# mpitid/babble

Hardware: AMD Instinct MI355X
Metric: consensus-ordered events/sec at N participants (higher is better)
Workload: dtype int32; 1 GPU; random-gossip DAG, 256 participants, 10000000 events per GPU, RunConsensus every K=256 events (39063 calls); participants=256, events_per_graph=10000000, k=256, graphs_per_gpu=1, parallelism=replicas1

## Files before the change

### babble_amd/csrc/hge_coords.hip

```cpp
#include <hip/hip_runtime.h>
#include <stdint.h>

namespace hge {

__global__ void k_la_clear(Tables t, const int32_t* olen, const int32_t* len, int32_t* zero,
                           int nzero) {
  const int j = blockIdx.y;
  const int N = t.N;
  if (j == 0 && blockIdx.x == 0)
    for (int i = threadIdx.x; i < nzero; i += blockDim.x) zero[i] = 0;
  const int64_t lo = (int64_t)olen[j] * N, hi = (int64_t)len[j] * N;
  int32_t* base = t.LA + (size_t)j * t.ccap * N;
  for (int64_t e = lo + (int64_t)blockIdx.x * blockDim.x + threadIdx.x; e < hi;
       e += (int64_t)gridDim.x * blockDim.x)
    base[e] = -1;
}

template <int NP>
__global__ void __launch_bounds__(256) k_la_sweep(Tables t, const int2* segs, int nseg, int SEG,
                                                  const int32_t* len, const int32_t* prev,
                                                  int32_t* changed) {
  constexpr int G = 256 / NP;
  constexpr int SEGMAX = 64;
  constexpr int U = 32;
// ... 443 lines not shown
    for (int h = 0; h < 16; h += CH) {
      int kv[CH];
#pragma unroll
      for (int i = 0; i < CH; i++) {
        const int jj = c0 + ty + 4 * (h + i), q = p0 + tx;
        if (jj < N && q < pend) {
          const FT f = FDT[((size_t)jj * N + a) * ccap + q];
          kv[i] = (sizeof(FT) == 2 && f == (FT)0xFFFF) ? INF32 : (int)f;
        } else {
          kv[i] = INF32;
        }
      }
      int64_t tv[CH];
      const bool tson = p0 + tx >= ts0 && p0 + tx < ts1;
#pragma unroll
      for (int i = 0; i < CH; i++) {
        const int jj = c0 + ty + 4 * (h + i);
        tv[i] = tson ? t.tsch[(size_t)(jj < N ? jj : 0) * ccap + (kv[i] != INF32 ? kv[i] : 0)] : own;
      }
#pragma unroll
      for (int i = 0; i < CH; i++) {
        tile[ty + 4 * (h + i)][tx] = kv[i];
        const int64_t d = tv[i] - own;
        const bool esc = d < -(int64_t)INT32_MAX || d > (int64_t)INT32_MAX;
        toff[ty + 4 * (h + i)][tx] = kv[i] == INF32 ? 0 : (esc ? INT32_MIN : (int32_t)d);
      }
    }
    }
    __syncthreads();
    const int NT = (N + 63) >> 6;
    for (int r = ty; r < 64; r += 4) {
      const int q = p0 + r, jj = c0 + tx;
      const bool tsrow = q >= ts0 && q < ts1;
      bool esc = false;
      if (q < pend && jj < N) {
        const size_t o = rowoff(t, a, q) + jj;
        const int32_t dv = toff[tx][r];
        esc = dv == INT32_MIN;
        if constexpr (sizeof(FT) == 2) {
          const int f = tile[tx][r];
          __builtin_nontemporal_store((uint16_t)(f == INF32 ? 0xFFFFu : (uint32_t)f + 1), t.FD16 + o);
        } else {
          __builtin_nontemporal_store(tile[tx][r], t.FD + o);
        }
        if (tsrow) __builtin_nontemporal_store(dv, t.FDTD + o);
      }
      const bool any = __ballot(esc) != 0;
      if (tx == 0 && q < pend && tsrow) t.FDTW[((size_t)a * ccap + q) * NT + by] = any ? 1 : 0;
    }
    __syncthreads();
  }
}

__global__ void k_fdt16_to32(const uint16_t* src, int32_t* dst, size_t n, int bias) {
  for (size_t i = (size_t)blockIdx.x * blockDim.x + threadIdx.x; i < n; i += (size_t)gridDim.x * blockDim.x)
    dst[i] = src[i] == 0xFFFFu ? INF32 : (int32_t)src[i] - bias;
}

__global__ void __launch_bounds__(256) k_fd_qlo(Tables t, const int32_t* olen, const int32_t* len, int32_t* qlo) {
  fd_qlo_body(t, olen, len, qlo, blockIdx.x);
}
__global__ void __launch_bounds__(256) k_chain_fill_qlo(Tables t, int n0, int n1, const UpEv* up, UpDst dst, int nfb,
                                                        const int32_t* olen, const int32_t* len, int32_t* qlo,
                                                        int32_t* fst, int32_t* zbar, uint64_t* zgran, int ngran) {
  if (fst && blockIdx.x == gridDim.x - 1) {
    frontier_start_body(t, olen, len, fst, nullptr, zbar, zgran, ngran);
  } else if ((int)blockIdx.x < nfb) {
    const int x = n0 + blockIdx.x * blockDim.x + threadIdx.x;
    if (x < n1) chain_fill_one(t, x, n0, up, dst);
  } else {
    fd_qlo_body(t, olen, len, qlo, blockIdx.x - nfb);
  }
}

}
```

### babble_amd/csrc/hge_engine.hip

```cpp
#include <hip/hip_runtime.h>

#include <algorithm>
#include <chrono>
#include <cstdio>
#include <cstdlib>
#include <cstring>
#include <mutex>
#include <optional>
#include <string>
#include <thread>
#include <utility>
#include <vector>

#include "../../include/hge.h"
#include "hge_plan.h"
#include "hge_kernels.hip"
#include "hge_wide32.hip"
#include "hge_coords.hip"
#include "hge_coords_win.hip"
#include "hge_rounds_coop.hip"
#include "hge_rounds_direct.hip"
#include "hge_walk_spec.hip"

using namespace hge;

#define HIPCHK(x)                                                                    \
  do {                                                                               \
    hipError_t e_ = (x);                                                             \
    if (e_ != hipSuccess) {                                                          \
      throw EngineError(HGE_ERR_DEVICE, std::string(#x) + ": " + hipGetErrorString(e_)); \
    }                                                                                \
  } while (0)

#define KLAUNCH_AS(name, kern, ...)                                                    \
  do {                                                                                 \
    hp.launches++;                                                                     \
    prof_begin(name);                                                                  \
    hipLaunchKernelGGL(kern, __VA_ARGS__);                                             \
    const hipError_t le_ = hipGetLastError();                                          \
    if (le_ != hipSuccess)                                                             \
      throw EngineError(HGE_ERR_DEVICE, std::string("launch ") + name + ": " + hipGetErrorString(le_)); \
    prof_end();                                                                        \
  } while (0)
#define KLAUNCH(kern, ...) KLAUNCH_AS(#kern, kern, __VA_ARGS__)

#define NW_T(B, kern, ...) KLAUNCH(kern<B>, __VA_ARGS__)
#define NW_PT(B, kern, ...) KLAUNCH((kern<B>), __VA_ARGS__)
#define NW_PAT(B, kern, A, ...) KLAUNCH((kern<A, B>), __VA_ARGS__)
#define NW_PATC(B, kern, A, C, ...) KLAUNCH((kern<A, B, C>), __VA_ARGS__)
#define NW_SWITCH_(nw, CASE1, SHAPE, ...)                          \
  switch (nw) {                                                    \
    CASE1                                                          \
    case 2:                                                        \
      SHAPE(2, __VA_ARGS__);                                       \
      break;                                                       \
    case 3:                                                        \
      SHAPE(3, __VA_ARGS__);                                       \
      break;                                                       \
    case 4:                                                        \
      SHAPE(4, __VA_ARGS__);                                       \
      break;                                                       \
    default:                                                       \
      throw EngineError(HGE_ERR_INTERNAL, "unsupported N");        \
  }
#define KLAUNCH_NW(nw, SHAPE, ...) NW_SWITCH_(nw, case 1 : SHAPE(1, __VA_ARGS__); break;, SHAPE, __VA_ARGS__)
#define KLAUNCH_NW2(nw, SHAPE, ...) NW_SWITCH_(nw, , SHAPE, __VA_ARGS__)

namespace {

// ... 88 lines not shown
    pin_ord = nullptr;
    pin_ord_dev = nullptr;
    pin_ord_cap = 0;
    HIPCHK(hipHostMalloc((void**)&pin_ord, std::max<size_t>(n, 1) * 4, hipHostMallocDefault));
    pin_ord_cap = std::max<size_t>(n, 1);
    void* dp = nullptr;
    pin_ord_dev = hipHostGetDevicePointer(&dp, pin_ord, 0) == hipSuccess ? (int32_t*)dp : nullptr;
  }
  int64_t n_und = 0;

  std::vector<int64_t> replay_calls;
  std::vector<int64_t> replay_counts;

  int64_t Ecap = 0;
  int ccap = 0, Rcap = 0;
  DBuf<int32_t> d_creator, d_index, d_sp, d_op, d_ntx, d_round, d_rr, d_und;
  DBuf<int64_t> d_ts, d_cts;
  DBuf<uint64_t> d_S;
  DBuf<uint8_t> d_coin, d_wit;
  DBuf<int32_t> d_chain, d_LA, d_FD, d_FSS;
  DBuf<int32_t> s_w32, s_w32a;
  DBuf<uint32_t> d_LA16;
  DBuf<int2> d_opcp;
  DBuf<int64_t> d_tsch;
  DBuf<int32_t> d_C, d_W, d_rcnt, d_minw;
  DBuf<uint64_t> d_ssb, d_seeb;
  DBuf<uint8_t> d_fame;
  DBuf<int32_t> s_small, s_newwit;
  DBuf<int32_t> s_LCR, s_clast;
  DBuf<uint8_t> s_dec, s_decbit;
  DBuf<int32_t> s_segcnt, s_segcall, s_seground, s_theta;
  DBuf<uint8_t> s_segdec;
  DBuf<uint64_t> s_segfws;
  DBuf<int32_t> s_recv, s_rr, s_fund, s_upos, s_und2, s_bpos, s_vis;
  bool vis_all = false;
  DBuf<int64_t> s_cts;
  DBuf<unsigned char> s_keys, s_keys2;
  DBuf<int32_t> s_part, s_fst, s_relay, s_rfail;
  DBuf<uint8_t> s_dec2;
  bool minw_full = true;
  int n_sweeps = 0;
  DBuf<int32_t> d_FDT, s_chg, s_bar, s_dirty;
  DBuf<int32_t> s_src;
  DBuf<int4> s_lwplan;
  DBuf<uint32_t> s_lwsum, s_lwinit;
  DBuf<int32_t> s_lwpos, s_lwrisky;
  int ncu_cache = 0;
  int n_cu() {
    if (!ncu_cache) HIPCHK(hipDeviceGetAttribute(&ncu_cache, hipDeviceAttributeMultiprocessorCount, device));
    return ncu_cache;
  }
  DBuf<int32_t> d_FDTD;
  DBuf<uint8_t> d_FDTW;
  DBuf<int32_t> d_WLA;
  DBuf<uint16_t> d_WLR;
  DBuf<uint64_t> d_ssc, s_gran;
  DBuf<int32_t> s_bseg;
  DBuf<uint64_t> s_H;
  DBuf<int32_t> s_hn, s_hres;
  uint32_t walk_epoch = 0;
  int walk_chk[2] = {448, 2};
  bool coop_checked = false;
  int coop_nb = 0, coop_ncu = 0, coop_spec_nb = -1, coop_spec_bs = 0;
  const void* coop_spec_fn() const {
    return coop_spec_bs == 1024 ? (const void*)k_rounds_coop_spec<1024> : (const void*)k_rounds_coop_spec<512>;
  }
  DBuf<uint64_t> s_cH, s_cS, s_cT, s_cM;
  DBuf<uint32_t> s_mb;
  DBuf<int32_t> s_cn;
  uint32_t coop_epoch = 0;

  hipEvent_t ev[8] = {};
  bool prof_on = false;
  std::vector<hipEvent_t> prof_pool;
  std::vector<std::pair<std::string, int>> prof_rec;
  std::vector<std::string> prof_names;
  std::vector<double> prof_ms;
  std::vector<int64_t> prof_cnt;
  int R_div = 0;
  std::vector<int32_t> h_minw;
  DBuf<int32_t> s_cctl, s_out;
  std::vector<int32_t> h_cctl;
  int64_t* c_nc = nullptr;
  int32_t *c_Rc = nullptr, *c_Lc = nullptr, *c_flags = nullptr, *c_pr = nullptr, *c_pidx = nullptr;
  int32_t* c_sgo = nullptr;
  const int32_t* segoff_p = nullptr;
  DBuf<int32_t> s_kctl;
  std::vector<int32_t> h_kctl;
  std::vector<hge_plan::Seg> h_segs;
  bool und_fresh = false;
  float stage_ms[7] = {};

  Tables tables() const {
    Tables t;
    t.N = N;
    t.NW = NW;
    t.SM = SM;
    t.ccap = ccap;
    t.Rcap = Rcap;
    t.creator = d_creator.p;
    t.index = d_index.p;
    t.sp = d_sp.p;
    t.op = d_op.p;
    t.ts = d_ts.p;
    t.S = d_S.p;
    t.coin = d_coin.p;
// ... 69 lines not shown
      while (k < prof_names.size() && prof_names[k] != r.first) k++;
      if (k == prof_names.size()) {
        prof_names.push_back(r.first);
        prof_ms.push_back(0);
        prof_cnt.push_back(0);
      }
      prof_ms[k] += ms;
      prof_cnt[k] += 1;
    }
    prof_rec.clear();
  }

  DBuf<uint64_t> s_dbg;
  bool dbg_on = getenv("HGE_STAMPS") != nullptr;
  uint64_t* dbg_p() {
    if (!dbg_on) return nullptr;
    if (!s_dbg.p) {
      s_dbg.need(16);
      HIPCHK(hipMemset(s_dbg.p, 0, 16 * 8));
    }
    return s_dbg.p;
  }
  void dbg_dump() {
    if (!dbg_on || !s_dbg.p) return;
    uint64_t v[16];
    readback(v, s_dbg.p, 16);
    fprintf(stderr, "[hge stamps]");
    for (int i = 0; i < 16; i++) fprintf(stderr, " %llu", (unsigned long long)v[i]);
    fprintf(stderr, "\n");
  }

  void destroy() {
    if (st) (void)hipStreamSynchronize(st);
    if (getenv("HGE_HOST_PHASES") && hp.calls) {
      const double c = (double)hp.calls;
      fprintf(stderr,
              "{\"hge_host_phases\": {\"calls\": %lld, \"launches_per_call\": %.2f, \"copies_per_call\": %.2f, "
              "\"insert_us\": %.2f, \"consensus_us\": %.2f, \"sync_wait_us\": %.2f}}\n",
              (long long)hp.calls, hp.launches / c, hp.copies / c, hp.insert_ns / c / 1e3, hp.call_ns / c / 1e3,
              hp.wait_ns / c / 1e3);
    }
    for (auto& e : ev)
      if (e) (void)hipEventDestroy(e);
    for (auto& e : prof_pool) (void)hipEventDestroy(e);
    prof_pool.clear();
    DBuf<int32_t>* i32s[] = {&d_creator, &d_index,  &d_sp,    &d_op,     &d_ntx,     &d_round,
                             &d_rr,      &d_und,    &d_chain, &d_LA,     &d_FD,      &d_C,
                             &d_W,       &d_rcnt,   &d_minw,  &s_small,  &s_newwit,  &s_LCR,
                             &s_clast,   &s_segcnt, &s_segcall, &s_seground, &s_theta,
                             &s_recv,    &s_rr,     &s_bpos,  &s_fund,   &s_upos,    &s_vis,
                             &s_und2,    &s_part,   &s_fst,    &d_FSS,
                             &d_FDT,     &s_chg,    &s_bar,   &s_bseg,   &s_kctl,    &s_cctl,
                             &s_out,     &s_hn,     &s_hres,  &s_dirty,  &d_WLA,     &s_lwpos,
                             &s_lwrisky, &s_src,    &s_relay, &s_rfail};
    for (auto* b : i32s) b->free_();
    s_dec2.free_();
    s_lwplan.free_();
    d_WLR.free_();
    s_xbuf.free_();
    s_sord.free_();
    s_soff.free_();
    s_lwsum.free_();
    s_lwinit.free_();
    d_ts.free_();
    d_FDTD.free_();
    d_FDTW.free_();
    d_cts.free_();
    s_cts.free_();
    d_S.free_();
    d_ssb.free_();
    d_seeb.free_();
    s_H.free_();
    s_wdbg.free_();
    s_segfws.free_();
    d_coin.free_();
    d_wit.free_();
    d_fame.free_();
    s_dec.free_();
    s_decbit.free_();
    s_segdec.free_();
    s_keys.free_();
    s_keys2.free_();
    d_opcp.free_();
    d_tsch.free_();
    d_LA16.free_();
    d_ssc.free_();
    s_gran.free_();
    s_cH.free_();
    s_cS.free_();
    s_cT.free_();
    s_cM.free_();
    s_cn.free_();
    s_mb.free_();
    s_hist.free_();
    s_hstate.free_();
    s_hssc.free_();
    if (pin) (void)hipHostFree(pin);
    pin = nullptr;
    pin_cap = pin_used = 0;
    if (pin_ord) (void)hipHostFree(pin_ord);
    pin_ord = nullptr;
    pin_ord_dev = nullptr;
    pin_ord_cap = 0;
    cons_pin_n = 0;
    if (st) (void)hipStreamDestroy(st);
    st = nullptr;
  }
// ... 333 lines not shown
    if (!bytes) return;
    char* q = pin_take(bytes);
    hp.copies++;
    HIPCHK(hipMemcpyAsync(q, dev, bytes, hipMemcpyDeviceToHost, st));
    pending.push_back({host, (size_t)(q - pin), bytes});
  }
  size_t d2h_pinned(const void* dev, size_t bytes) {
    char* q = pin_take(bytes);
    if (bytes) hp.copies++;
    if (bytes) HIPCHK(hipMemcpyAsync(q, dev, bytes, hipMemcpyDeviceToHost, st));
    return (size_t)(q - pin);
  }
  int64_t n_syncs = 0;
  struct HostPhases {
    int64_t calls = 0, launches = 0, copies = 0, wait_ns = 0, call_ns = 0, insert_ns = 0;
  } hp;
  static int64_t now_ns() {
    return std::chrono::duration_cast<std::chrono::nanoseconds>(
               std::chrono::steady_clock::now().time_since_epoch()).count();
  }
  void sync() {
    n_syncs++;
    const int64_t w0 = now_ns();
    HIPCHK(hipStreamSynchronize(st));
    hp.wait_ns += now_ns() - w0;
    for (const Pending& pd : pending) memcpy(pd.dst, pin + pd.off, pd.bytes);
    pending.clear();
    pin_used = 0;
  }
  template <typename F>
  void readback(F* host, const F* dev, size_t n) {
    d2h(host, dev, n * sizeof(F));
    sync();
  }

  struct CoordStep {
    bool fresh = false;
    int64_t n0 = 0, n1 = 0;
    int maxnew = 0;
    int tot0 = 0;
    int SEG = 0, nseg = 0;
    int maxlen = 0, minlen = 0;
    enum class La { Windows, Seq, Sweeps } la = La::Sweeps;
    int32_t *rstate = nullptr, *olen = nullptr, *len = nullptr, *plo = nullptr, *qlo = nullptr;
    int32_t *fss_lo = nullptr, *fss_off = nullptr, *fss_total = nullptr, *segbase = nullptr;
    const int2* segs = nullptr;
    int32_t *cand_lo = nullptr, *cand_hi = nullptr;
    int32_t* risky1 = nullptr;
    const UpEv* up = nullptr;
    UpDst up_dst{};
    bool frontier_started = false;
    bool qlo_done = false;
    bool fd_done = false;
    bool take_frontier_start() { return std::exchange(frontier_started, false); }
  };
  std::optional<CoordStep> cstep;
  struct Walk {
    bool assigned = false;
    bool tail_done = false;
    const int32_t* err_src = nullptr;
    bool host_err = false;
  };
  void bind_kctl(CoordStep& s, const hge_plan::CoordsCtl& L) const {
    int32_t* p = s_kctl.p;
    s.rstate = p + L.rstate, s.olen = p + L.olen(), s.len = p + L.nlen();
    s.plo = p + L.plo, s.qlo = p + L.qlo;
    s.fss_lo = p + L.fss_lo(), s.fss_off = p + L.fss_off(), s.fss_total = p + L.fss_total();
    s.segs = (const int2*)(p + L.segs), s.segbase = p + L.segbase;
    s.cand_lo = split_on() ? p + L.cand_lo() : nullptr;
    s.cand_hi = split_on() ? p + L.cand_hi() : nullptr;
    s.risky1 = p + L.risky;
    s.up = L.up_words ? (const UpEv*)(p + L.up) : nullptr;
  }
  std::chrono::steady_clock::time_point w_start;
  bool ext_on = false, ext_natural = false;
  int ext_rows = 0;
  std::vector<int32_t> ext_C;
  std::vector<uint64_t> ext_ssc;
  DBuf<int32_t> s_hist, s_hstate;
  DBuf<uint64_t> s_hssc;
  struct SplitPlan {
    int part = 0, nparts = 0;
    std::vector<int64_t> a;
    std::vector<int32_t> cb;
    std::vector<int64_t> clo;
  } sp;
  bool sp_active = false;
  bool split_on() const { return sp_active && sp.nparts > 1; }
  hge_exchange_fn x_fn = nullptr;
  void* x_ctx = nullptr;
  bool rec_on = false, rec_have = false;
  std::vector<std::vector<uint8_t>> rec_dec;
  std::vector<int32_t> rec_order, rec_rr, rec_left;
  std::vector<int64_t> rec_counts, rec_cts;
  int x_iter = 0;
  DBuf<uint8_t> s_xbuf;
  bool emulating() const { return split_on() && !x_fn && rec_have; }
  DBuf<int32_t> s_sord;
  DBuf<int64_t> s_soff;
  void* x_buf(int64_t bytes) {
    sync();
    if (emulating()) {
      s_xbuf.need((size_t)bytes * sp.nparts);
      return s_xbuf.p;
    }
    void* b = nullptr;
// ... 15 lines not shown
        if ((int64_t)h_minw[pr_round[mid]] < ev) lo = mid + 1;
        else hi = mid;
      }
      return lo;
    };
    win_lo = g == 0 ? 0 : first_at(sp.a[g]);
    win_hi = g == sp.nparts - 1 ? nr : first_at(sp.a[g + 1]);
  }
  int32_t mnr_pre = 0;
  int64_t mnr_key[3] = {-1, 0, 0};
  void coords() {
    if (coords_a()) coords_b();
  }
  int npow() const { return N <= 64 ? 64 : N <= 128 ? 128 : 256; }
  int wit_group() const {
    int G = 1;
    while (G < std::min(N, 64)) G <<= 1;
    return G;
  }

  bool coords_a() {
    cstep.reset();
    upload();
    if (wide32_pending) to_wide32();
    if (n_events == n_coords) return false;
    CoordStep s;
    plan_step(s);
    const Tables t = tables();
    chain_fill(t, s);
    last_ancestors(t, s);
    first_descendants(t, s);
    cstep = s;
    return true;
  }
  void plan_step(CoordStep& s) {
    s.n0 = n_coords;
    s.n1 = n_events;
    s.SEG = N <= 32 ? 16 : 64;
    s.la = sweep16() && la_windows() ? CoordStep::La::Windows
           : la_seq_ok(s.n1 - s.n0)  ? CoordStep::La::Seq
                                     : CoordStep::La::Sweeps;
    const bool sweeps = s.la == CoordStep::La::Sweeps;
    h_segs.clear();
    if (sweeps) hge_plan::sweep_segments(h_segs, coords_len, chain_len, s.SEG);
    s.nseg = sweeps ? (int)h_segs.size() : 1;
    s.fresh = R == 0;
    s.minlen = INT32_MAX;
    for (int c = 0; c < N; c++) {
      s.maxnew = std::max(s.maxnew, chain_len[c] - coords_len[c] + 1);
      s.fresh = s.fresh && coords_len[c] == 0;
      s.maxlen = std::max(s.maxlen, chain_len[c]);
      s.minlen = std::min(s.minlen, chain_len[c]);
    }
    std::vector<int32_t> cand;
    if (split_on()) {
      const int64_t A = sp.clo[sp.part], B = sp.a[sp.part + 1];
      cand.resize(2 * (size_t)N);
      for (int c = 0; c < N; c++) {
        const std::vector<int32_t>& ch = h_chain[c];
        cand[c] = (int)(std::lower_bound(ch.begin(), ch.end(), (int32_t)A) - ch.begin());
        cand[N + c] = (int)(std::lower_bound(ch.begin(), ch.end(), (int32_t)B) - ch.begin());
      }
    }
    const bool packed = up_n0 == s.n0 && up_n1 == s.n1;
    if (packed && h_up.empty()) throw EngineError(HGE_ERR_INTERNAL, "packed upload without records");
    static_assert(sizeof(UpEv) % 4 == 0, "records are whole words");
    static_assert(sizeof(hge_plan::Seg) == sizeof(int2), "the kernels read segments as int2");
    const hge_plan::CoordsCtl L =
        hge_plan::coords_ctl_layout(N, h_segs.size(), packed ? sizeof(UpEv) * h_up.size() / 4 : 0);
    s.tot0 = hge_plan::fill_coords_ctl(h_kctl, L, R, coords_len, chain_len, h_segs, s.SEG, cand);
    if (packed) memcpy(&h_kctl[L.up], h_up.data(), sizeof(UpEv) * h_up.size());
    s_kctl.need(h_kctl.size());
    h2d(s_kctl.p, h_kctl.data(), 4 * h_kctl.size());
    bind_kctl(s, L);
    s.up_dst = UpDst{d_creator.p, d_index.p, d_sp.p, d_op.p, d_ntx.p, d_ts.p, d_S.p, d_coin.p};
    up_n0 = up_n1 = -1;
    h_up.clear();
  }
  void chain_fill(const Tables& t, CoordStep& s) {
    if (s.la == CoordStep::La::Seq) return;
    const int nfb = div_up((int)(s.n1 - s.n0), 256);
    if (!s.fresh && N <= 256) {
      const bool fst = N > 32 && !wide32 && !frontier_fallback && !split_on() && !ext_on;
      if (fst) {
        s_fst.need(N + 1);
        s_bar.need(2);
        s_gran.need(2 * (size_t)N);
      }
      KLAUNCH(k_chain_fill_qlo, dim3(nfb + N + (fst ? 1 : 0)), dim3(256), 0, st, t, (int)s.n0, (int)s.n1,
              s.up, s.up_dst, nfb, (const int32_t*)s.olen, (const int32_t*)s.len, s.qlo,
              fst ? s_fst.p : (int32_t*)nullptr, fst ? s_bar.p : (int32_t*)nullptr,
              fst ? (uint64_t*)s_gran.p : (uint64_t*)nullptr, 2 * N);
      s.frontier_started = fst;
      s.qlo_done = true;
    } else {
      KLAUNCH(k_chain_fill, dim3(nfb), dim3(256), 0, st, t, (int)s.n0, (int)s.n1, s.up, s.up_dst);
    }
  }
  RoundAssign round_assign(const CoordStep& s, bool tail) {
    s_newwit.need(s.n1 - s.n0);
    RoundAssign ra{(int)s.n0, (int)s.n1, s_newwit.p, s.rstate + 2, und_appended ? d_und.p + n_und : (int32_t*)nullptr};
    if (tail) {
      ra.minw = d_minw.p;
      ra.G = wit_group();
      ra.und = d_und.p;
      ra.n_und = (int)n_und;
// ... 373 lines not shown
    }
    return hres[1];
  }
  void wide_walk(Tables t, const CoordStep& s, int32_t rlo, const int32_t* rlo_dev, int Rprev) {
    const int32_t* FDT = d_FDT.p;
    const int32_t* olen = s.olen;
    const int32_t* len = s.len;
    int32_t* rstate = s.rstate;
    int32_t* err = s_bar.p + 1;
    uint64_t* gran = s_gran.p;
    uint64_t* ssc = d_ssc.p;
    uint64_t* dbg = dbg_p();
    if (direct_rounds()) {
      s_mb.need((size_t)npow() * npow());
      uint32_t* mb = s_mb.p;
      const int32_t* nostart = nullptr;
      int32_t* nohist = nullptr;
      int hmax = 0, extra = 0;
      const char* hs = getenv("HGE_TEST_HANDOFF_STALL");
      int stall_ep = hs ? atoi(hs) : 0;
      void* dargs[] = {&t, &olen, &len, &rstate, &rlo, &rlo_dev, &Rprev, &gran, &err, &ssc, &mb, &dbg,
                       &nostart, &nohist, &hmax, &nostart, &extra, &stall_ep};
      prof_begin("k_rounds_direct");
      HIPCHK(launch_resident(direct_fn(), dim3(N), dim3(1024), dargs));
      prof_end();
    } else {
      void* args[] = {&t, &FDT, &olen, &len, &rstate, &rlo, &rlo_dev, &Rprev, &gran, &err, &ssc, &dbg};
      prof_begin("k_rounds_coop");
      HIPCHK(launch_resident((const void*)k_rounds_coop, dim3(N), dim3(COOP_BS), args));
      prof_end();
    }
    if (getenv("HGE_TEST_HANDOFF_FAIL")) {
      const int32_t one = 1, down = hge_plan::kRoundsStoodDown;
      h2d(err, &one, 4);
      h2d(rstate + 1, &down, 4);
    }
  }
  const void* direct_fn() const {
    return N <= 64 ? (const void*)k_rounds_direct<1024, 64>
         : N <= 128 ? (const void*)k_rounds_direct<1024, 128>
                    : (const void*)k_rounds_direct<1024, 256>;
  }

  bool sweep16() const { return N > 32 && !wide32; }
  bool wla16() const { return N > 192 && (N & 3) == 0 && !wide32; }

  void to_wide32() {
    auto test_stop = [&](int stage) {
      if (test_w32_fail == stage) {
        test_w32_fail = 0;
        throw EngineError(HGE_ERR_DEVICE, "test: to_wide32 stopped after stage " + std::to_string(stage));
      }
    };
    if (!(w32_done & 4)) {
      grow_chain_table(d_LA, ccap, false);
      w32_done |= 4;
      test_stop(1);
    }
    if (fdt16()) {
      const size_t n = (size_t)N * N * ccap;
      for (int which = 0; which < 2; which++) {
        if (w32_done & (1 << which)) continue;
        DBuf<int32_t>& b = which ? d_FD : d_FDT;
        int32_t* q = nullptr;
        HIPCHK(hipMalloc(&q, sizeof(int32_t) * n));
        KLAUNCH(k_fdt16_to32, dim3((unsigned)std::min<size_t>(div_up(n, 256), 65536)), dim3(256), 0, st,
                (const uint16_t*)b.p, q, n, which);
        sync();
        b.free_();
        b.p = q;
        b.n = n;
        w32_done |= 1 << which;
        test_stop(2 + which);
      }
    }
    s_w32.need(N);
    h2d(s_w32.p, coords_len.data(), 4 * (size_t)N);
    wide32 = true;
    wide32_pending = false;
    w32_done = 0;
    Tables t = tables();
    int64_t most = 1;
    for (int c = 0; c < N; c++) most = std::max<int64_t>(most, (int64_t)coords_len[c] * N);
    KLAUNCH(k_la16_to_la32, dim3((unsigned)std::min<int64_t>(div_up(most, 256), 4096), N), dim3(256), 0, st, t,
            (const uint32_t*)d_LA16.p, (const int32_t*)s_w32.p);
  }

  Walk rounds_step32(const CoordStep& s) {
    Tables t = tables();
    s_fst.need(N + 1);
    KLAUNCH(k_frontier_start, dim3(1), dim3(256), 0, st, t, s.olen, s.len, s_fst.p, (int32_t*)nullptr,
            (int32_t*)nullptr, (uint64_t*)nullptr, 0);
    int32_t rlo = INF32;
    readback(&rlo, s_fst.p, 1);
    if (rlo == INF32) return {};
    const int Rprev = R, NB = 32;
    s_w32a.need(NB);
    for (int r = rlo;;) {
      HIPCHK(hipMemsetAsync(s_w32a.p, 0, 4 * NB, st));
      int k = 0;
      for (; k < NB && r + k + 1 < Rcap; k++)
        KLAUNCH(k_round_step32, dim3(N), dim3(256), 0, st, t, (const int32_t*)s.olen, (const int32_t*)s.len,
                r + k, Rprev, d_ssc.p, s_w32a.p + k);
      std::vector<int32_t> alive(NB, 0);
      readback(alive.data(), s_w32a.p, NB);
      for (int q = 0; q < k; q++)
// ... 111 lines not shown
    const int nseg = s.nseg, SEG = s.SEG, maxnew = s.maxnew;
    const bool p16 = sweep16();
    if (p16) s_dirty.need(nseg);
    int32_t* dirty = p16 ? s_dirty.p : nullptr;
    if (p16)
      KLAUNCH(k_la_clear16, dim3(std::max(1, std::min(64, div_up((int64_t)maxnew * t.NW2, 256))), N),
              dim3(256), 0, st, t, olen, len, s_chg.p, MAXSW, dirty, nseg);
    else
      KLAUNCH(k_la_clear, dim3(std::max(1, std::min(64, div_up((int64_t)maxnew * N, 256))), N),
              dim3(256), 0, st, t, olen, len, s_chg.p, MAXSW);
    const int NPt = p16 ? (t.NW2 <= 32 ? 32 : t.NW2 <= 64 ? 64 : 128)
                        : (N <= 16 ? 16 : N <= 32 ? 32 : N <= 64 ? 64 : N <= 128 ? 128 : 256);
    int sw = 0;
    for (int group = 12;; group = 8) {
      for (int g = 0; g < group; g++, sw++) {
        if (sw >= MAXSW) throw EngineError(HGE_ERR_INTERNAL, "lastAncestors sweeps did not converge");
        const int32_t* prev = sw > 0 ? s_chg.p + sw - 1 : nullptr;
        if (p16) {
          switch (NPt) {
#define SW16(NPV)                                                                                \
  case NPV:                                                                                      \
    KLAUNCH(k_la_sweep16<NPV>, dim3(div_up(nseg, 256 / NPV)), dim3(256), 0, st, t, s.segs, nseg, \
            SEG, len, prev, s_chg.p + sw, olen, s.segbase, dirty, sw);                          \
    break;
            SW16(32)
            SW16(64)
            SW16(128)
#undef SW16
          }
        } else {
          switch (NPt) {
#define SW(NPV)                                                                                  \
  case NPV:                                                                                      \
    KLAUNCH(k_la_sweep<NPV>, dim3(div_up(nseg, 256 / NPV)), dim3(256), 0, st, t, s.segs, nseg,   \
            SEG, len, prev, s_chg.p + sw);                                                       \
    break;
            SW(16)
            SW(32)
            SW(64)
            SW(128)
            SW(256)
#undef SW
          }
        }
      }
      std::vector<int32_t> flags(sw);
      readback(flags.data(), s_chg.p, sw);
      if (!flags[sw - 1]) {
        n_sweeps = (int)(std::find(flags.begin(), flags.end(), 0) - flags.begin()) + 1;
        break;
      }
    }
  }
  void first_descendants(const Tables& t, const CoordStep& s) {
    if (s.fd_done) return;
    const int32_t* olen = s.olen;
    const int32_t* len = s.len;
    const int maxnew = s.maxnew;
    if (fdt16()) {
      KLAUNCH((k_la16_rows_runs<uint16_t>), dim3(div_up(maxnew + 1, 64), div_up(N, 64), N), dim3(256), 0, st, t,
              (uint16_t*)d_FDT.p, s.plo, olen, len);
    } else if (sweep16()) {
      KLAUNCH((k_la16_rows_runs<int32_t>), dim3(div_up(maxnew + 1, 64), div_up(N, 64), N), dim3(256), 0, st, t,
              d_FDT.p, s.plo, olen, len);
    } else {
      KLAUNCH((k_la16_rows_runs<int32_t, true>), dim3(div_up(maxnew + 1, 64), div_up(N, 64), N), dim3(256), 0,
              st, t, d_FDT.p, s.plo, olen, len);
    }
    int span = 1;
    if (!s.fresh) {
      if (!s.qlo_done) KLAUNCH(k_fd_qlo, dim3(N), dim3(256), 0, st, t, olen, len, s.qlo);
      span = maxnew + 64;
    } else {
      span = std::max(span, s.maxlen);
    }
    if (fdt16())
      KLAUNCH((k_fd_transpose_ts<uint16_t>), dim3(N, div_up(N, 64), std::min(div_up(span, 64), 65535)), dim3(256),
              0, st, t, (const uint16_t*)d_FDT.p, s.qlo, len, (const int32_t*)s.cand_lo,
              (const int32_t*)s.cand_hi);
    else if (N > 16)
      KLAUNCH((k_fd_transpose_ts<int32_t>), dim3(N, div_up(N, 64), std::min(div_up(span, 64), 65535)), dim3(256),
              0, st, t, (const int32_t*)d_FDT.p, s.qlo, len, (const int32_t*)s.cand_lo,
              (const int32_t*)s.cand_hi);
    else
      KLAUNCH(k_transpose, dim3(div_up(span, 64), div_up(N, 64), N), dim3(256), 0, st, t, d_FDT.p,
              (int32_t*)nullptr, s.qlo, len, 1);
  }


  enum class OrderRan {
    Stages,
    CallFront,
    CallTail,
  };
  struct Batch {
    const int64_t* calls = nullptr;
    int ncalls = 0;
    bool do_fame = false, do_order = false, commit = false;
    std::vector<int32_t>* order_out = nullptr;
    std::vector<int64_t>* counts_out = nullptr;
    std::vector<int32_t> Rc;
    bool fresh_und = false;
    bool ord = false;
    bool spl = false;
    int32_t* cand = nullptr;
    int ncand = 0;
    int rr_lo = 0, R_last = 0, nr = 0;
    hge_plan::ResultsLayout out;
    hge_plan::FameWindows w;
    hge_plan::CtlLayout ctl;
    int64_t nslot = 0;
    bool hdr_done = false;
    bool lcr_dev = false;
    int lcr_new = -1, c_set = -1;
    bool lcr_up = false;
    std::optional<FameCall> fame_pending;
    SegInfo si{};
    OrderRan order_ran = OrderRan::Stages;
    bool wla_done = false;
    bool got_order = false;
    bool wrote_direct = false;
    bool split_done = false;
  };
  int32_t* out_counts() const { return s_out.p + hge_plan::ResultsLayout::kCounts; }
  int32_t* out_ids(const Batch& b) const { return s_out.p + b.out.ids; }
  unsigned long long* out_tx(const Batch& b) const { return (unsigned long long*)(s_out.p + b.out.o_tx); }
  int32_t* out_word(size_t k) const { return s_out.p + k; }
  const int32_t* lcr_src(const Batch& b) const { return b.lcr_dev ? (const int32_t*)(c_flags + 1) : nullptr; }
  void out_init(const Batch& b) {
    const int nh = (int)b.out.header();
    KLAUNCH(k_out_init, dim3(div_up(nh, 256)), dim3(256), 0, st, s_out.p, nh, lcr_src(b));
  }
  void bind_ctl(const hge_plan::CtlLayout& L) {
    c_nc = (int64_t*)s_cctl.p;
    c_Rc = s_cctl.p + L.Rc;
    c_Lc = s_cctl.p + L.Lc;
    c_flags = s_cctl.p + L.flags;
    c_pr = s_cctl.p + L.pr;
    c_pidx = s_cctl.p + L.pidx;
    c_sgo = s_cctl.p + L.sgo;
  }

  void consensus_batch(const std::vector<int64_t>& calls, bool do_fame, bool do_order, bool commit,
                       std::vector<int32_t>* order_out, std::vector<int64_t>* counts_out) {
    if (calls.empty()) return;
    int64_t tp[5] = {now_ns(), 0, 0, 0, 0};
    Batch b;
    b.calls = calls.data();
    b.ncalls = (int)calls.size();
    b.do_fame = do_fame;
    b.do_order = do_order;
    b.commit = commit;
    b.order_out = order_out;
    b.counts_out = counts_out;
    prologue(b, calls);
    tp[1] = now_ns();
    decide_fame(b);
    tp[2] = now_ns();
    if (b.ord) {
      order_stages(b);
      bucket_and_sort(b);
    } else {
      s_out.need(b.out.total());
      launch_pending_fame(b);
      if (!b.hdr_done) out_init(b);
    }
    if (b.fame_pending) throw EngineError(HGE_ERR_INTERNAL, "DecideFame's launch left pending");
    persist_fame(b);
    if (b.spl && b.got_order) {
      split_commit(s_out.p, out_counts(), out_ids(b), b.out.ntxb, out_tx(b), order_out, counts_out);
      b.got_order = false;
      b.split_done = true;
    }
    tp[3] = now_ns();
    close_batch(b);
    tp[4] = now_ns();
    if (b.ncalls > 1000 && getenv("HGE_HOST_PHASES")) phases_line(tp);
    prof_collect();
  }
  void phases_line(const int64_t* tp) const {
    fprintf(stderr, "[hge consensus] prologue %.3f ms, fame %.3f ms (incl. syncs), order enqueue %.3f ms, closing %.3f ms\n",
            (tp[1] - tp[0]) / 1e6, (tp[2] - tp[1]) / 1e6, (tp[3] - tp[2]) / 1e6, (tp[4] - tp[3]) / 1e6);
  }

  void prologue(Batch& b, const std::vector<int64_t>& calls) {
    consensus_sync();
    x_iter = 0;
    b.Rc = hge_plan::rounds_at_calls(calls, h_minw);
    b.fresh_und = und_fresh;
    und_fresh = false;
    b.ord = b.do_order && n_und > 0;
    b.ncand = (int)n_und;
    b.cand = d_und.p;
    b.spl = split_on() && b.ord && b.fresh_und;
    if (b.spl) {
      b.cand = d_und.p + sp.clo[sp.part];
      b.ncand = (int)(sp.a[sp.part + 1] - sp.clo[sp.part]);
    }
    int32_t mnr = 0;
    const bool pre = mnr_key[0] >= 0 && !b.spl && n_divided == mnr_key[2] &&
                     n_und == mnr_key[0] + (mnr_key[2] - mnr_key[1]);
    mnr_key[0] = -1;
    if (b.ord && !b.fresh_und && pre) {
      mnr = mnr_pre;
    } else if (b.ord && (!b.fresh_und || b.spl)) {
      h2d(s_small.p + 7, &kInf, 4);
      KLAUNCH(k_min_round, dim3(div_up(b.ncand, 256)), dim3(256), 0, st, d_round.p, b.cand, b.ncand,
              s_small.p + 7);
      readback(&mnr, s_small.p + 7, 1);
    }
    b.rr_lo = mnr + 1;
    b.R_last = b.spl ? b.Rc[sp.cb[sp.part + 1] - 1] : b.Rc[b.ncalls - 1];
    b.nr = b.ord ? std::max(0, b.R_last - b.rr_lo) : 0;
    b.out = hge_plan::results_layout(b.ncalls, b.ord ? b.ncand : 0);
  }

  FameCall fame_call_args(const Batch& b, int32_t* hdr) const {
    const int nrounds = b.w.nrounds();
    FameCall f{};
    f.pr_round = c_pr;
    f.pr_off = c_pr + nrounds;
    f.pr_cf = c_pr + 2 * nrounds;
    f.pr_len = c_pr + 3 * nrounds;
    f.nrounds = nrounds;
    f.npairs = b.w.npairs;
    f.nc = c_nc;
// ... 577 lines not shown
    readback(r.data(), d_round.p + lo, r.size());
    for (size_t k = 0; k < ids.size(); k++) out[k] = r[ids[k] - lo];
  }

  void scan_large(const int32_t* in, int32_t* out, int n, int32_t* total) {
    if (n <= 16384) {
      KLAUNCH(k_scan_small, dim3(1), dim3(1024), 0, st, in, out, n, total);
      return;
    }
    const int nb = div_up(n, 1024);
    s_part.need(2 * (size_t)nb + 2);
    KLAUNCH(k_scan_blocks, dim3(nb), dim3(256), 0, st, in, out, n, s_part.p);
    KLAUNCH(k_scan_small, dim3(1), dim3(1024), 0, st, s_part.p, s_part.p + nb, nb, total);
    KLAUNCH(k_scan_add, dim3(div_up(n, 256)), dim3(256), 0, st, out, n, s_part.p + nb);
  }

  int group_lanes() const { return N <= 16 ? 16 : N <= 32 ? 32 : 64; }

  void fame_decide(const Tables& t, const hge_plan::FameWindows& w, int npairs, bool timeline = true) {
    const int nrounds = w.nrounds();
    int win_lo = 0, win_hi = nrounds;
    if (split_on()) split_rounds_of(sp.part, w.round, win_lo, win_hi);
    const int p0 = win_lo < nrounds ? w.off[win_lo] : npairs;
    const int p1 = win_hi < nrounds ? w.off[win_hi] : npairs;
    if (p1 > p0 && N == 64 * NW) {
      KLAUNCH_NW(NW, NW_PT, k_fame_decide_blk, dim3(p1 - p0), dim3(N), 0, st, t, c_pr + win_lo,
                 c_pr + nrounds + win_lo, c_pr + 2 * nrounds + win_lo, win_hi - win_lo, p0, p1, c_nc, c_Rc, s_dec.p,
                 (const int32_t*)nullptr);
    } else if (p1 > p0) {
      KLAUNCH_NW(NW, NW_PT, k_fame_decide, dim3(div_up((p1 - p0) * N, 256)), dim3(256), 0, st, t, c_pr + win_lo,
                 c_pr + nrounds + win_lo, c_pr + 2 * nrounds + win_lo, win_hi - win_lo, p0, p1, c_nc, c_Rc, s_dec.p);
    }
    if (split_on()) split_exchange_dec(w.round, w.off, npairs);
    if (!timeline) return;
    const int G = group_lanes();
    const dim3 tgrid(div_up((int64_t)nrounds * G, 256));
    const int32_t *pr_off = c_pr + nrounds, *pr_cf = c_pr + 2 * nrounds, *pr_len = c_pr + 3 * nrounds;
    if (G == 16) {
      KLAUNCH((k_fame_timeline_g<16, 1>), tgrid, dim3(256), 0, st, t, c_pr, pr_off, pr_cf, pr_len, nrounds, c_nc,
              s_dec.p, s_decbit.p, c_Lc);
    } else if (G == 32) {
      KLAUNCH((k_fame_timeline_g<32, 1>), tgrid, dim3(256), 0, st, t, c_pr, pr_off, pr_cf, pr_len, nrounds, c_nc,
              s_dec.p, s_decbit.p, c_Lc);
    } else {
      KLAUNCH_NW(NW, NW_PAT, k_fame_timeline_g, 64, tgrid, dim3(256), 0, st, t, c_pr, pr_off, pr_cf, pr_len,
                 nrounds, c_nc, s_dec.p, s_decbit.p, c_Lc);
    }
  }
  void fame_persist(const Tables& t, int nrounds) {
    KLAUNCH(k_fame_persist, dim3(div_up((int64_t)nrounds * N, 256)), dim3(256), 0, st, t, c_pr, c_pr + nrounds,
            c_pr + 2 * nrounds, c_pr + 3 * nrounds, nrounds, s_clast.p, s_dec.p);
  }

  void recv_dispatch(Batch& b) {
    const bool wmed = N > 16;
    const bool ident = b.fresh_und && b.cand == d_und.p && (int64_t)b.ncand == n_events;
    int32_t* bseg = nullptr;
    if (wmed) {
      s_bseg.need(b.ncand);
      bseg = s_bseg.p;
      ensure_wla(b);
    }
    const Tables t = tables();
    KLAUNCH_NW(NW, NW_T, k_round_received, dim3(div_up(b.ncand, 256)), dim3(256), 0, st, t, b.cand, b.ncand,
               vis_all ? (const int32_t*)nullptr : (const int32_t*)s_vis.p, b.ncalls, 0, b.rr_lo, b.R_last,
               segoff_p, s_segcnt.p, s_segcall.p, s_segdec.p, s_segfws.p, s_theta.p, s_recv.p, s_rr.p, s_cts.p,
               bseg);
    if (wmed)
      KLAUNCH_NW(NW, NW_T, k_median_wave, dim3(div_up(b.ncand, 4 * MED_EPW)), dim3(256), 0, st, t,
                 ident ? (const int32_t*)nullptr : b.cand, b.ncand, s_recv.p, s_rr.p, bseg, s_segfws.p, s_cts.p);
  }

  bool dividing = false, und_appended = false;
  void divide() {
    dividing = true;
    und_appended = false;
    try {
      coords();
    } catch (...) {
      dividing = false;
      throw;
    }
    dividing = false;
    if (n_divided < n_coords) {
      const int64_t a = n_divided, m = n_coords - n_divided;
      ensure_events(n_coords);
      if (!und_appended) KLAUNCH(k_iota, dim3(div_up(m, 256)), dim3(256), 0, st, d_und.p + n_und, m, (int32_t)a);
      n_und += m;
      n_divided = n_coords;
    }
    update_rdiv();
  }

  bool online_fast(std::vector<int32_t>& order) {
    const int64_t n0 = n_coords, n1 = n_events, m = n1 - n0;
    if (N > 16 || m <= 0 || R == 0 || cstep || split_on() || rec_on || ext_on || sp_active) return false;
    if (n_divided != n0 || !la_seq_ok(m) || n_und + m > 65536 || n_und + m > SCAN_LDS) return false;
    if (getenv("HGE_NO_ONLINE_FAST")) return false;
    if (*std::max_element(chain_len.begin(), chain_len.end()) + 1 >= 0xFFFF) return false;
    consensus_sync();
    ensure_rcap((int64_t)R + m + 4);
    dividing = true;
    und_appended = false;
    if (!coords_a()) {
      dividing = false;
      throw EngineError(HGE_ERR_INTERNAL, "online call: no coordinates to compute");
    }
    if (!cstep || !cstep->frontier_started)
      throw EngineError(HGE_ERR_INTERNAL, "online call: frontier start not fused");
    CoordStep s = *cstep;
    cstep.reset();
    walk_online(s);
    dividing = false;
    n_coords = n1;
    coords_len = chain_len;
    n_und += m;
    n_divided = n_coords;
    und_fresh = false;
    const int Rmax = R + (int)m + 1;
    const int nround_max = std::max(1, Rmax - 2 - lcr), nr_max = std::max(1, Rmax);
    Batch b;
    b.calls = &n_divided;
    b.ncalls = 1;
// ... 251 lines not shown
  h->consensus.clear();
  h->cons_pin_n = 0;
  h->n_und = 0;
  h->ext_on = false;
  h->w_start = std::chrono::steady_clock::now();
  h->reset_rounds();
  HIPCHK(hipEventRecord(h->ev[0], h->st));
  h->coords_a();
}

static void replay_end(hge_engine* h, int64_t* n_ordered) {
  const int64_t keep = h->n_events;
  if (h->cstep) h->coords_b();
  HIPCHK(hipEventRecord(h->ev[1], h->st));
  const auto w1 = std::chrono::steady_clock::now();
  h->n_divided = keep;
  h->update_rdiv();
  if (keep > 0) h->fill_iota(h->d_und.p, keep, 0);
  h->n_und = keep;
  h->und_fresh = keep > 0;
  h->replay_counts.clear();
  h->lazy_order = h->pin_ord_cap >= (size_t)keep;
  try {
    h->consensus_batch(h->replay_calls, true, true, true, nullptr, &h->replay_counts);
  } catch (...) {
    h->lazy_order = false;
    throw;
  }
  h->lazy_order = false;
  HIPCHK(hipEventRecord(h->ev[2], h->st));
  HIPCHK(hipEventSynchronize(h->ev[2]));
  const auto w2 = std::chrono::steady_clock::now();
  float a = 0, b = 0;
  HIPCHK(hipEventElapsedTime(&a, h->ev[0], h->ev[1]));
  HIPCHK(hipEventElapsedTime(&b, h->ev[1], h->ev[2]));
  auto ms = [](std::chrono::steady_clock::time_point x, std::chrono::steady_clock::time_point y) {
    return (float)std::chrono::duration<double, std::milli>(y - x).count();
  };
  h->stage_ms[0] = a;
  h->stage_ms[1] = ms(h->w_start, w1);
  h->stage_ms[2] = ms(w1, w2);
  h->stage_ms[3] = b;
  h->stage_ms[4] = ms(h->w_start, w2);
  h->stage_ms[6] = a + b;
  if (n_ordered) *n_ordered = h->consensus_size();
  h->dbg_dump();
}

int hge_replay_run(hge_engine* h, int64_t* n_ordered) {
  GUARD_BEGIN
  REFUSE_IF_FAILED(h)
  h->sp_active = false;
  if (h->rec_on) h->rec_dec.clear();
  replay_begin(h);
  replay_end(h, n_ordered);
  if (h->rec_on) {
    const int64_t E = h->n_events;
    h->consensus_sync();
    h->rec_order = h->consensus;
    h->rec_counts = h->replay_counts;
    h->rec_rr.resize(E);
    h->rec_cts.resize(E);
    h->readback(h->rec_rr.data(), h->d_rr.p, (size_t)E);
    h->readback(h->rec_cts.data(), h->d_cts.p, (size_t)E);
    h->rec_left.resize(h->n_und);
    if (h->n_und) h->readback(h->rec_left.data(), h->d_und.p, (size_t)h->n_und);
    h->rec_on = false;
    h->rec_have = true;
  }
  return HGE_OK;
  GUARD_END(h)
}

int hge_split_plan(hge_engine* h, int32_t part, int32_t nparts, const int64_t* ev_bounds,
                   const int32_t* call_bounds, const int64_t* cand_lo) {
  if (!h) return HGE_ERR_ARG;
  GUARD_BEGIN
  if (nparts <= 1) {
    h->sp = hge_engine::SplitPlan();
    return HGE_OK;
  }
  auto bad = [&](const char* why) {
    h->err = std::string("hge_split_plan: ") + why;
    return HGE_ERR_ARG;
  };
  if (h->N <= 32 || !h->direct_rounds() || h->wide32 || h->wide32_pending)
    return bad("needs the wide direct rounds path (N > 32, N % 4 == 0, chains below 65,535 events)");
  if (part < 0 || part >= nparts || !ev_bounds || !call_bounds || !cand_lo) return bad("bad argument");
  const int64_t E = h->n_events;
  const int ncalls = (int)h->replay_calls.size();
  if (ev_bounds[0] != 0 || ev_bounds[nparts] != E || call_bounds[0] != 0 || call_bounds[nparts] != ncalls)
    return bad("the bounds must cover the staged stream and its calls");
  for (int g = 0; g < nparts; g++) {
    if (ev_bounds[g + 1] < ev_bounds[g] || call_bounds[g + 1] <= call_bounds[g])
      return bad("bounds must ascend and every part needs a call");
    if (cand_lo[g] < 0 || cand_lo[g] > ev_bounds[g] || cand_lo[g] >= ev_bounds[g + 1])
      return bad("cand_lo[p] must lie in [0, ev_bounds[p]] below ev_bounds[p + 1]");
  }
  if (E > INT32_MAX) return bad("stream too long");
  h->sp.part = part;
  h->sp.nparts = nparts;
  h->sp.a.assign(ev_bounds, ev_bounds + nparts + 1);
  h->sp.cb.assign(call_bounds, call_bounds + nparts + 1);
  h->sp.clo.assign(cand_lo, cand_lo + nparts);
  return HGE_OK;
  GUARD_END(h)
}
// ... 670 lines not shown
```

Before: 188.0 million events/s.

## Defer FD timestamp transpose and fuse median computation into row-tiled kernel

During bulk replay, a lighter k_fd_rows16 transpose now writes only the FD16 rows and skips the timestamp-delta (FDTD) table. That table is marked stale and rebuilt lazily, either for undetermined events only (fdtd_tail) or fully when another path needs it. A new k_median_rows kernel computes the consensus-timestamp medians from FD16 row tiles, gathering timestamps in place of the precomputed FDTD deltas. The aim is to cut memory traffic from writing and re-reading the full FDTD table, at the cost of extra state tracking and gather loads inside the median kernel.

```diff
diff --git a/babble_amd/csrc/hge_coords.hip b/babble_amd/csrc/hge_coords.hip
--- a/babble_amd/csrc/hge_coords.hip
+++ b/babble_amd/csrc/hge_coords.hip
@@ -519,6 +519,43 @@
   }
 }
 
+__global__ void __launch_bounds__(256) k_fd_rows16(Tables t, const uint16_t* FDT, const int32_t* plo,
+                                                   const int32_t* len) {
+  __shared__ uint16_t tile[64][66];
+  const int N = t.N;
+  const size_t ccap = t.ccap;
+  const int64_t nbk = (int64_t)gridDim.x * gridDim.y * gridDim.z;
+  const int64_t lb = xcd_block(blockIdx.x + (int64_t)gridDim.x * (blockIdx.y + (int64_t)gridDim.y * blockIdx.z), nbk);
+  const int bx = (int)(lb % gridDim.x), by = (int)((lb / gridDim.x) % gridDim.y), bz = (int)(lb / ((int64_t)gridDim.x * gridDim.y));
+  const int a = bx;
+  const int pend = len[a];
+  const int c0 = by * 64;
+  const int tx = threadIdx.x & 63, ty = threadIdx.x >> 6;
+  const int pb = plo[a] & ~3;
+  const int qd = threadIdx.x & 15, r0 = threadIdx.x >> 4;
+  for (int p0 = pb + bz * 64; p0 < pend; p0 += gridDim.z * 64) {
+    uint2 w[4];
+#pragma unroll
+    for (int h = 0; h < 4; h++) {
+      const int jj = c0 + r0 + 16 * h, q = p0 + 4 * qd;
+      w[h] = (jj < N && q < pend) ? *(const uint2*)(FDT + ((size_t)jj * N + a) * ccap + q) : make_uint2(~0u, ~0u);
+    }
+#pragma unroll
+    for (int h = 0; h < 4; h++) {
+      const uint32_t u[4] = {w[h].x & 0xFFFFu, w[h].x >> 16, w[h].y & 0xFFFFu, w[h].y >> 16};
+#pragma unroll
+      for (int e = 0; e < 4; e++)
+        tile[r0 + 16 * h][4 * qd + e] = (u[e] == 0xFFFFu || p0 + 4 * qd + e >= pend) ? (uint16_t)0xFFFFu : (uint16_t)(u[e] + 1);
+    }
+    __syncthreads();
+    for (int r = ty; r < 64; r += 4) {
+      const int q = p0 + r, jj = c0 + tx;
+      if (q < pend && jj < N) __builtin_nontemporal_store(tile[tx][r], t.FD16 + rowoff(t, a, q) + jj);
+    }
+    __syncthreads();
+  }
+}
+
 __global__ void k_fdt16_to32(const uint16_t* src, int32_t* dst, size_t n, int bias) {
   for (size_t i = (size_t)blockIdx.x * blockDim.x + threadIdx.x; i < n; i += (size_t)gridDim.x * blockDim.x)
     dst[i] = src[i] == 0xFFFFu ? INF32 : (int32_t)src[i] - bias;
diff --git a/babble_amd/csrc/hge_engine.hip b/babble_amd/csrc/hge_engine.hip
--- a/babble_amd/csrc/hge_engine.hip
+++ b/babble_amd/csrc/hge_engine.hip
@@ -15,6 +15,7 @@
 #include "../../include/hge.h"
 #include "hge_plan.h"
 #include "hge_kernels.hip"
+#include "hge_median_rows.hip"
 #include "hge_wide32.hip"
 #include "hge_coords.hip"
 #include "hge_coords_win.hip"
@@ -209,6 +210,11 @@
   }
   DBuf<int32_t> d_FDTD;
   DBuf<uint8_t> d_FDTW;
+  bool rows_bulk = false;
+  bool fdtd_stale = false;
+  int fdtd_maxlen = 0;
+  DBuf<int32_t> s_fdlo;
+  bool test_rows_fallback = getenv("HGE_TEST_MEDIAN_ROWS_FALLBACK") != nullptr;
   DBuf<int32_t> d_WLA;
   DBuf<uint16_t> d_WLR;
   DBuf<uint64_t> d_ssc, s_gran;
@@ -384,7 +390,7 @@
                              &s_und2,    &s_part,   &s_fst,    &d_FSS,
                              &d_FDT,     &s_chg,    &s_bar,   &s_bseg,   &s_kctl,    &s_cctl,
                              &s_out,     &s_hn,     &s_hres,  &s_dirty,  &d_WLA,     &s_lwpos,
-                             &s_lwrisky, &s_src,    &s_relay, &s_rfail};
+                             &s_lwrisky, &s_src,    &s_relay, &s_rfail,  &s_fdlo};
     for (auto* b : i32s) b->free_();
     s_dec2.free_();
     s_lwplan.free_();
@@ -824,6 +830,7 @@
     bool frontier_started = false;
     bool qlo_done = false;
     bool fd_done = false;
+    bool fd_rows_only = false;
     bool take_frontier_start() { return std::exchange(frontier_started, false); }
   };
   std::optional<CoordStep> cstep;
@@ -945,6 +952,7 @@
       s.maxlen = std::max(s.maxlen, chain_len[c]);
       s.minlen = std::min(s.minlen, chain_len[c]);
     }
+    s.fd_rows_only = rows_bulk && s.fresh && s.n0 == 0 && fdt16() && !split_on() && !rec_on && !ext_on;
     std::vector<int32_t> cand;
     if (split_on()) {
       const int64_t A = sp.clo[sp.part], B = sp.a[sp.part + 1];
@@ -1424,6 +1432,7 @@
         throw EngineError(HGE_ERR_DEVICE, "test: to_wide32 stopped after stage " + std::to_string(stage));
       }
     };
+    ensure_fdtd();
     if (!(w32_done & 4)) {
       grow_chain_table(d_LA, ccap, false);
       w32_done |= 4;
@@ -1641,8 +1650,22 @@
       }
     }
   }
+  void fdtd_pass(const char* name, int zgrid) {
+    const Tables t = tables();
+    KLAUNCH_AS(name, (k_fd_transpose_ts<uint16_t>), dim3(N, div_up(N, 64), std::max(1, std::min(zgrid, 65535))),
+               dim3(256), 0, st, t, (const uint16_t*)d_FDT.p, (const int32_t*)s_fdlo.p,
+               (const int32_t*)(s_fdlo.p + N), (const int32_t*)nullptr, (const int32_t*)nullptr);
+  }
+  void ensure_fdtd() {
+    if (!fdtd_stale) return;
+    if (!fdt16()) throw EngineError(HGE_ERR_INTERNAL, "stale FD timestamp rows past the uint16 runs");
+    HIPCHK(hipMemsetAsync(s_fdlo.p, 0, 4 * (size_t)N, st));
+    fdtd_pass("fdtd_ensure (k_fd_transpose_ts<uint16_t>)", div_up(std::max(fdtd_maxlen, 1), 64));
+    fdtd_stale = false;
+  }
   void first_descendants(const Tables& t, const CoordStep& s) {
     if (s.fd_done) return;
+    if (!s.fresh) ensure_fdtd();
     const int32_t* olen = s.olen;
     const int32_t* len = s.len;
     const int maxnew = s.maxnew;
@@ -1663,7 +1686,15 @@
     } else {
       span = std::max(span, s.maxlen);
     }
-    if (fdt16())
+    if (s.fresh) fdtd_stale = false;
+    if (s.fd_rows_only) {
+      KLAUNCH(k_fd_rows16, dim3(N, div_up(N, 64), std::min(div_up(span, 64), 65535)), dim3(256), 0, st, t,
+              (const uint16_t*)d_FDT.p, (const int32_t*)s.qlo, len);
+      s_fdlo.need(2 * (size_t)N);
+      h2d(s_fdlo.p + N, chain_len.data(), 4 * (size_t)N);
+      fdtd_maxlen = s.maxlen;
+      fdtd_stale = true;
+    } else if (fdt16())
       KLAUNCH((k_fd_transpose_ts<uint16_t>), dim3(N, div_up(N, 64), std::min(div_up(span, 64), 65535)), dim3(256),
               0, st, t, (const uint16_t*)d_FDT.p, s.qlo, len, (const int32_t*)s.cand_lo,
               (const int32_t*)s.cand_hi);
@@ -1761,6 +1792,7 @@
       b.got_order = false;
       b.split_done = true;
     }
+    fdtd_tail(b);
     tp[3] = now_ns();
     close_batch(b);
     tp[4] = now_ns();
@@ -2444,6 +2476,20 @@
             c_pr + 2 * nrounds, c_pr + 3 * nrounds, nrounds, s_clast.p, s_dec.p);
   }
 
+  void fdtd_tail(const Batch& b) {
+    if (!fdtd_stale) return;
+    if (!b.got_order || b.spl || !b.commit) {
+      ensure_fdtd();
+      return;
+    }
+    HIPCHK(hipMemcpyAsync(s_fdlo.p, s_fdlo.p + N, 4 * (size_t)N, hipMemcpyDeviceToDevice, st));
+    KLAUNCH(k_und_low, dim3(std::max(1, std::min(div_up(b.ncand, 256), 1024))), dim3(256), 0, st,
+            (const int32_t*)d_creator.p, (const int32_t*)d_index.p, (const int32_t*)d_und.p,
+            (const int32_t*)out_word(hge_plan::ResultsLayout::kUndetermined), s_fdlo.p);
+    fdtd_pass("fdtd_tail (k_fd_transpose_ts<uint16_t>)", std::min(div_up(std::max(fdtd_maxlen, 1), 64), 4));
+    fdtd_stale = false;
+  }
+
   void recv_dispatch(Batch& b) {
     const bool wmed = N > 16;
     const bool ident = b.fresh_und && b.cand == d_und.p && (int64_t)b.ncand == n_events;
@@ -2458,9 +2504,17 @@
                vis_all ? (const int32_t*)nullptr : (const int32_t*)s_vis.p, b.ncalls, 0, b.rr_lo, b.R_last,
                segoff_p, s_segcnt.p, s_segcall.p, s_segdec.p, s_segfws.p, s_theta.p, s_recv.p, s_rr.p, s_cts.p,
                bseg);
-    if (wmed)
+    if (wmed && ident && fdtd_stale && !test_rows_fallback) {
+      constexpr int TQ = 16, NT = 512;
+      const int64_t nb = (int64_t)N * div_up(fdtd_maxlen, TQ);
+      KLAUNCH_AS("k_median_rows<16, 512>", (k_median_rows<TQ, NT>), dim3((unsigned)nb), dim3(NT),
+                 sizeof(int32_t) * TQ * (N + 4), st, t, (const int32_t*)(s_fdlo.p + N), (const int32_t*)s_recv.p,
+                 (const int32_t*)s_rr.p, (const int32_t*)bseg, (const uint64_t*)s_segfws.p, s_cts.p);
+    } else if (wmed) {
+      ensure_fdtd();
       KLAUNCH_NW(NW, NW_T, k_median_wave, dim3(div_up(b.ncand, 4 * MED_EPW)), dim3(256), 0, st, t,
                  ident ? (const int32_t*)nullptr : b.cand, b.ncand, s_recv.p, s_rr.p, bseg, s_segfws.p, s_cts.p);
+    }
   }
 
   bool dividing = false, und_appended = false;
@@ -2818,7 +2872,13 @@
   REFUSE_IF_FAILED(h)
   h->sp_active = false;
   if (h->rec_on) h->rec_dec.clear();
+  struct Bulk {
+    hge_engine* h;
+    ~Bulk() { h->rows_bulk = false; }
+  } bulk{h};
+  h->rows_bulk = true;
   replay_begin(h);
+  h->rows_bulk = false;
   replay_end(h, n_ordered);
   if (h->rec_on) {
     const int64_t E = h->n_events;
diff --git a/babble_amd/csrc/hge_median_rows.hip b/babble_amd/csrc/hge_median_rows.hip
--- /dev/null
+++ b/babble_amd/csrc/hge_median_rows.hip
@@ -0,0 +1,169 @@
+#pragma once
+
+namespace hge {
+
+template <int TQ, int NT>
+__global__ void __launch_bounds__(NT) k_median_rows(Tables t, const int32_t* len, const int32_t* recv_call,
+                                                    const int32_t* rr_in, const int32_t* bseg,
+                                                    const uint64_t* seg_fws, int64_t* cts_out) {
+  constexpr int NWV = NT / 64;
+  constexpr int RPW = TQ / NWV;
+  constexpr int PER = 256 * TQ / NT;
+  constexpr int LDP = 256 * TQ / 4 / NT;
+  static_assert(TQ % NWV == 0 && RPW <= 8 && (256 * TQ) % (4 * NT) == 0 && NT % TQ == 0, "tile shape");
+  extern __shared__ __attribute__((aligned(16))) int32_t s_tile[];
+  __shared__ __attribute__((aligned(16))) int s_mhist[NWV][256];
+  __shared__ int64_t s_own[TQ];
+  __shared__ int s_x[TQ], s_rr[TQ], s_sg[TQ], s_wide[TQ];
+  const int N = t.N, NW = t.NW;
+  const size_t ccap = t.ccap;
+  const int tid = threadIdx.x, lane = tid & 63, wv = tid >> 6;
+  const int64_t lb = xcd_block(blockIdx.x, gridDim.x);
+  const int c = (int)(lb % N), q0 = (int)(lb / N) * TQ;
+  const int pend = len[c];
+  if (q0 >= pend) return;
+  const int rows = min(TQ, pend - q0);
+  const int RS16 = N + 2;
+  const int RS32 = N + 4;
+  const uint16_t* src = t.FD16 + rowoff(t, c, q0);
+  const int npiece = rows * (N >> 2);
+  uint2 pw[LDP];
+#pragma unroll
+  for (int i = 0; i < LDP; i++) {
+    const int p = tid + NT * i;
+    pw[i] = p < npiece ? *(const uint2*)(src + 4 * (size_t)p) : make_uint2(~0u, ~0u);
+  }
+  int lv = 0;
+  if (tid < TQ) {
+    const int q = q0 + tid;
+    int x = 0, rr = 0, sg = 0;
+    int64_t own = 0;
+    if (q < pend) {
+      x = t.chain[(size_t)c * ccap + q];
+      own = t.tsch[(size_t)c * ccap + q];
+      const int rc = recv_call[x], rr0 = rr_in[x], sg0 = bseg[x];
+      lv = rc >= 0;
+      rr = lv ? rr0 : 0;
+      sg = lv ? sg0 : 0;
+    }
+    s_x[tid] = lv ? x : -1;
+    s_rr[tid] = rr;
+    s_sg[tid] = sg;
+    s_own[tid] = own;
+    s_wide[tid] = 0;
+  }
+  uint16_t* const t16 = (uint16_t*)s_tile;
+#pragma unroll
+  for (int i = 0; i < LDP; i++) {
+    const int p = tid + NT * i;
+    if (p < npiece) {
+      const int e = 4 * p, q = e / N, j = e - q * N;
+      uint32_t* d = (uint32_t*)(t16 + q * RS16 + j);
+      d[0] = pw[i].x;
+      d[1] = pw[i].y;
+    }
+  }
+  if (!__syncthreads_or(lv)) return;
+  const int l4 = min(lane, (N >> 2) - 1);
+  int th[RPW][4];
+  uint32_t fw[RPW];
+#pragma unroll
+  for (int k = 0; k < RPW; k++) {
+    const int r = wv + NWV * k;
+    const bool on = s_x[r] >= 0;
+    const size_t o = ((size_t)(on ? s_rr[r] : 0) * N + c) * N + 4 * l4;
+    if (t.WLA16) {
+      const uint2 tw = *(const uint2*)(t.WLA16 + o);
+      th[k][0] = (int)(tw.x & 0xFFFFu) - 1;
+      th[k][1] = (int)(tw.x >> 16) - 1;
+      th[k][2] = (int)(tw.y & 0xFFFFu) - 1;
+      th[k][3] = (int)(tw.y >> 16) - 1;
+    } else {
+      const int4 tw = *(const int4*)(t.WLA + o);
+      th[k][0] = tw.x;
+      th[k][1] = tw.y;
+      th[k][2] = tw.z;
+      th[k][3] = tw.w;
+    }
+    fw[k] = (uint32_t)(seg_fws[(size_t)(on ? s_sg[r] : 0) * NW + min(lane >> 4, NW - 1)] >> ((4 * lane) & 63)) & 15u;
+  }
+  int kv[PER];
+#pragma unroll
+  for (int i = 0; i < PER; i++) {
+    const int idx = tid + NT * i, q = idx % TQ, j = idx / TQ;
+    const uint32_t v = (j < N && q < rows) ? t16[q * RS16 + j] : 0xFFFFu;
+    kv[i] = v == 0xFFFFu ? INF32 : (int)v - 1;
+  }
+  __syncthreads();
+  constexpr int GB = PER < 8 ? PER : 8;
+#pragma unroll
+  for (int h = 0; h < PER; h += GB) {
+    int64_t tv[GB];
+#pragma unroll
+    for (int i = 0; i < GB; i++) {
+      const int j = (tid + NT * (h + i)) / TQ;
+      tv[i] = kv[h + i] != INF32 ? t.tsch[(size_t)(j < N ? j : 0) * ccap + kv[h + i]] : 0;
+    }
+#pragma unroll
+    for (int i = 0; i < GB; i++) {
+      const int idx = tid + NT * (h + i), q = idx % TQ, j = idx / TQ;
+      if (j < N) {
+        const int64_t dlt = tv[i] - s_own[q];
+        const bool esc = kv[h + i] != INF32 && (dlt < -(int64_t)INT32_MAX || dlt > (int64_t)INT32_MAX);
+        s_tile[q * RS32 + j] = kv[h + i] == INF32 ? 0 : (int32_t)dlt;
+        if (esc) s_wide[q] = 1;
+      }
+    }
+  }
+  uint32_t inm = 0;
+#pragma unroll
+  for (int k = 0; k < RPW; k++) {
+    const int ix = q0 + wv + NWV * k;
+#pragma unroll
+    for (int e = 0; e < 4; e++)
+      if (4 * lane + e < N && ((fw[k] >> e) & 1u) && th[k][e] >= ix) inm |= 1u << (4 * k + e);
+  }
+  __syncthreads();
+#pragma unroll
+  for (int k = 0; k < RPW; k++) {
+    const int r = wv + NWV * k;
+    const int x = __builtin_amdgcn_readfirstlane(s_x[r]);
+    if (x < 0) continue;
+    const int ix = q0 + r;
+    const int4 ow = *(const int4*)(s_tile + r * RS32 + 4 * l4);
+    const int32_t o4[4] = {ow.x, ow.y, ow.z, ow.w};
+    bool in[4];
+#pragma unroll
+    for (int e = 0; e < 4; e++) in[e] = (inm >> (4 * k + e)) & 1u;
+    int64_t med;
+    if (!__builtin_amdgcn_readfirstlane(s_wide[r])) {
+      uint32_t v[4];
+#pragma unroll
+      for (int e = 0; e < 4; e++) v[e] = in[e] ? ((uint32_t)o4[e] ^ 0x80000000u) : ~0u;
+      med = s_own[r] + (int64_t)(int32_t)(wave_upper_median32_r8<4>(v, in, s_mhist[wv]) ^ 0x80000000u);
+    } else {
+      const size_t rw = (size_t)c * ccap + ix;
+      uint64_t v[4];
+#pragma unroll
+      for (int e = 0; e < 4; e++) {
+        const int dd = min(4 * lane + e, N - 1);
+        const int f = fd_at(t, rw, dd);
+        const int64_t ts = f != INF32 ? t.tsch[(size_t)dd * ccap + f] : 0;
+        v[e] = in[e] ? ((uint64_t)ts ^ 0x8000000000000000ull) : ~0ull;
+      }
+      med = wave_upper_median<4>(v, in);
+    }
+    if (lane == 0) cts_out[x] = med;
+  }
+}
+
+__global__ void k_und_low(const int32_t* creator, const int32_t* index, const int32_t* und, const int32_t* n_und,
+                          int32_t* lo) {
+  const int n = *n_und;
+  for (int i = blockIdx.x * blockDim.x + threadIdx.x; i < n; i += gridDim.x * blockDim.x) {
+    const int x = und[i];
+    atomicMin(&lo[creator[x]], index[x]);
+  }
+}
+
+}
```

Result: faster. 197.7 million events/s (median of 6 runs) (+5.1%).
